# tomwhite/disq

Measured on AMD Instinct MI355X. Metric: decompressed BAM GB/s + reads/sec (whole node) at 1/2/4/8 MI355X, higher is better.
Workload: dtype u8

## Files before the change

disq_amd/csrc/dq_api.hip:

```cpp
#include <hip/hip_runtime.h>

#include <fcntl.h>
#include <sys/stat.h>
#include <unistd.h>

#include <algorithm>
#include <chrono>
#include <cstdio>
#include <cstdlib>
#include <cstring>
#include <map>
#include <string>
#include <thread>
#include <type_traits>
#include <sys/mman.h>
#include <mutex>
#include <vector>

#include "../../include/disq_gpu.h"
#include "dq_internal.h"
#include "dq_sam_core.h"
#include "dq_vcf_core.h"
#include "dq_vcf_gt_core.h"
#include "dq_vcf_info_core.h"
// ... 644 lines not shown
    launch_exclusive_scan_i32(ctx->blk_us.as<int32_t>(), ctx->uoff.as<int64_t>(), nblk,
                              ctx->tmp.as<int64_t>(), s);
    if ((rc = get_i64(ctx, ctx->uoff.as<int64_t>() + nblk, &ulen))) return rc;
  }
  dbg(s, "chain", nblk, broken);
  ctx->nblk = nblk;
  if (nblk == 0 && L > 0) RET(DQ_EFORMAT, "no BGZF blocks found");
  ctx->ulen = ulen;
  HIPCHK(hipEventRecord(ctx->ev[1], s));
  if ((rc = ensure_all(ctx, ctx->U, (size_t)ulen + 256))) return rc;
  if ((rc = ensure_all(ctx, ctx->status, sizeof(int32_t) * (size_t)(nblk + 1)))) return rc;
  HIPCHK(hipMemsetAsync(ctx->status.p, 0, sizeof(int32_t) * (size_t)(nblk + 1), s));
  HIPCHK(hipMemsetAsync(ctx->U.as<uint8_t>() + ulen, 0, 256, s));
  {
    const uint32_t* crc_init = inflate3_tables(ctx->o.device);
    if (!crc_init) RET(DQ_EDEVICE, "CRC32 table initialisation failed on this device");
    static const bool timing = getenv("DQ_TIMING") != nullptr;
    uint64_t* tim = nullptr;
    if (timing) {
      HIPCHK(hipMalloc(&tim, sizeof(uint64_t) * 48 * (size_t)std::max<int64_t>(1, nblk)));
      HIPCHK(hipMemsetAsync(tim, 0, sizeof(uint64_t) * 48 * (size_t)std::max<int64_t>(1, nblk), s));
    }
    HIPCHK(hipEventRecord(ctx->ev[5], s));
    if ((rc = ensure_all(ctx, ctx->tails, INFLATE_TAIL_BYTES * (size_t)std::max<int64_t>(1, nblk)))) return rc;
    launch_inflate3(ctx->cbuf(), ctx->blk_pos.as<int64_t>(), ctx->blk_cs.as<int32_t>(),
                    ctx->blk_us.as<int32_t>(), ctx->uoff.as<int64_t>(), nblk, ctx->U.as<uint8_t>(),
                    ctx->status.as<int32_t>(), ctx->o.verify_crc, crc_init, tim, s, nullptr, 0,
                    ctx->tails.p);
    HIPCHK(hipEventRecord(ctx->ev[6], s));
    if (timing) {
      std::vector<uint64_t> h(48 * (size_t)nblk);
      HIPCHK(hipMemcpyAsync(h.data(), tim, 8 * h.size(), hipMemcpyDeviceToHost, s));
      HIPCHK(hipStreamSynchronize(s));
      (void)hipFree(tim);
      double acc[24] = {0};
      for (int64_t i = 0; i < nblk; i++)
        for (int k = 0; k < 24; k++) acc[k] += (double)h[32 * (size_t)i + k];
      static const char* nm[16] = {"header", "tables", "spec", "rounds", "scan", "emit",
                                   "resolve+store", "crc", "hdr_read_lengths", "resolve_hop_next", "redo_rounds", "tables_build",
                                   "resolve_steps_jumps", "resolve_store", "resolve_jump_tail", "res_batches"};
      fprintf(stderr, "[dq] inflate3 phase cycles per BGZF block (thread 0, s_memtime):");
      for (int k = 0; k < 16; k++)
        if (nm[k][0] != '-') fprintf(stderr, " %s=%.0f", nm[k], acc[k] / (double)std::max<int64_t>(1, nblk));
      fprintf(stderr, "\n");
      const double nb = (double)std::max<int64_t>(1, nblk);
      fprintf(stderr, "[dq] first deflate block: header=%.0f tables=%.0f spec=%.0f rounds=%.0f emit=%.0f; "
              "later ones: header=%.0f tables=%.0f spec=%.0f rounds=%.0f emit=%.0f; deflate blocks per "
// ... 1002 lines not shown
      if (j0 >= nblk || bp[(size_t)j0] != a) RET(DQ_EFORMAT, ".bai chunk does not start at a BGZF block");
      const int64_t jc = std::upper_bound(bp.begin(), bp.end(), e) - bp.begin();
      const int64_t j1 = std::min(nblk, jc + extra);
      if (!win.empty() && j0 <= win.back().j1 + GAP) {
        W& w = win.back();
        w.jc = std::max(w.jc, jc);
        w.j1 = std::max(w.j1, j1);
      } else {
        win.push_back({j0, jc, j1, ub[k]});
      }
    }
    std::vector<int32_t> sel;
    for (const W& w : win)
      for (int64_t j = std::max<int64_t>(w.j0, sel.empty() ? 0 : sel.back() + 1); j < w.j1; j++)
        sel.push_back((int32_t)j);
    const int64_t nsel = (int64_t)sel.size();
    HIPCHK(hipEventRecord(ctx->ev[5], s));
    if (nsel) {
      if ((rc = ensure_all(ctx, ctx->sel, 4 * (size_t)nsel))) return rc;
      HIPCHK(hipMemcpyAsync(ctx->sel.p, sel.data(), 4 * (size_t)nsel, hipMemcpyHostToDevice, s));
      HIPCHK(hipMemsetAsync(ctx->status.p, 0, sizeof(int32_t) * (size_t)(nblk + 1), s));
      const uint32_t* crc_init = inflate3_tables(ctx->o.device);
      if (!crc_init) RET(DQ_EDEVICE, "CRC32 table initialisation failed on this device");
      if ((rc = ensure_all(ctx, ctx->tails, INFLATE_TAIL_BYTES * (size_t)nsel))) return rc;
      launch_inflate3(ctx->cbuf(), ctx->blk_pos.as<int64_t>(), ctx->blk_cs.as<int32_t>(),
                      ctx->blk_us.as<int32_t>(), ctx->uoff.as<int64_t>(), nblk, ctx->U.as<uint8_t>(),
                      ctx->status.as<int32_t>(), ctx->o.verify_crc, crc_init, nullptr, s,
                      ctx->sel.as<int32_t>(), nsel, ctx->tails.p);
    }
    HIPCHK(hipEventRecord(ctx->ev[6], s));
    {
      unsigned long long* d_bad = reinterpret_cast<unsigned long long*>(ctx->scal.as<char>() + 144);
      HIPCHK(hipMemsetAsync(d_bad, 0xff, 8, s));
      if (nsel) launch_first_bad(ctx->status.as<int32_t>(), ctx->sel.as<int32_t>(), nsel, d_bad, s);
      unsigned long long bad = 0;
      HIPCHK(hipMemcpyAsync(&bad, d_bad, 8, hipMemcpyDeviceToHost, s));
      HIPCHK(hipStreamSynchronize(s));
      if (bad != ~0ull) {
        int32_t st = 0;
        HIPCHK(hipMemcpy(&st, ctx->status.as<int32_t>() + bad, 4, hipMemcpyDeviceToHost));
        char msg[256];
        snprintf(msg, sizeof msg, "%s in BGZF block at %lld", status_name(st),
                 (long long)(bp[(size_t)bad] + ctx->base));
        RET(DQ_EFORMAT, msg);
      }
    }
    const int64_t SEG = 64 * 1024;
// ... 2906 lines not shown
```

disq_amd/csrc/dq_inflate3.hip:

```cpp
#include "dq_inflate_core.h"
#include "dq_internal.h"

#include <mutex>
#include <vector>

namespace dq {
namespace {

using namespace dqi;

#define DQ_HD __device__ __host__ __attribute__((always_inline)) inline

#ifndef DQ_BLK_WG
#define DQ_BLK_WG 512
#endif
constexpr int WG = DQ_BLK_WG;
static_assert(WG % 128 == 0 && WG >= 512 && WG <= 1024, "whole waves on every SIMD");
constexpr int NWV = WG / 64;
constexpr int NDEC = WG;
constexpr uint32_t OV_DEFAULT = 96;
#ifndef DQ_TAIL_OV
#define DQ_TAIL_OV OV_DEFAULT
#endif
constexpr int OUTCAP = 65536 + 24;
// ... 46 lines not shown
enum : int32_t { F_EXIT = 0, F_EOB = 1, F_ERR = 2, F_END = 3 };

constexpr int TOUT = 4096;
constexpr int TAIL_MAX_BITS = 32768;
constexpr int TW = 4;
#ifndef DQ_ROOT_REG
#define DQ_ROOT_REG 1
#endif
#ifndef DQ_TAIL_HDR1
#define DQ_TAIL_HDR1 1
#endif
constexpr int T_NCK = 4;
#ifndef DQ_TAIL_SEG
#define DQ_TAIL_SEG 96
#endif
constexpr int TAIL_SEG_MIN = DQ_TAIL_SEG;
constexpr int TIM_W = 32;
struct TailDesc {
  int32_t pos;
  int32_t produced;
  uint32_t crc_raw;
  int32_t flag;
};

struct alignas(16) LdsI {
  static constexpr int kLSUB = T_LSUB, kDROOT = T_DROOT, kDSUB = T_DSUB;
  [[maybe_unused]] static constexpr int kTEND = T_END;
  static constexpr bool kPair = true;
  alignas(8) uint32_t bm[2048];
  union {
    struct {
      uint16_t T[T_END];
      HuffCanon hl, hd;
      uint16_t lend[16], dend[16];
      uint16_t lent[288];
      uint16_t dent[32];
      union {
        uint16_t pair[1 << LR];
        struct {
          uint8_t lens[320];
          uint8_t clen[20];
          uint16_t clt[128];
          union {
            struct {
              int32_t cntw[NWV];
              int32_t cnts[NWV];
// ... 25 lines not shown
    struct {
      int32_t wsum[16];
      int32_t small[8 * 7];
    };
    uint32_t scratch[16 + 8 * 7];
  };
  alignas(16) uint8_t out[OUTCAP];
};
static_assert(sizeof(((LdsI*)nullptr)->scratch) >= 64 * 4, "one emit dummy word per lane");
static_assert(offsetof(LdsI, out) < 65536 - 4096, "the tables' offsets fit the DS offset field");
static_assert(2 * sizeof(LdsI) <= 160 * 1024, "two workgroups per CU");
static_assert(HB_WORDS * 4 <= T_END * 2, "header staging fits the decode table");

__device__ inline uint32_t* emit_dummy(LdsI& L) { return L.scratch; }

__constant__ uint32_t c_crc4[4][256];
__constant__ uint32_t c_x2n[32];
__constant__ uint32_t c_x8n[TOUT + 1];
constexpr int CRC_SL = 4 * (((65536 / 4 + WG - 1) / WG) | 1);
static_assert(CRC_SL * WG >= 65536, "the slices cover the largest block");
__constant__ uint32_t c_slice_shift[WG];
__constant__ uint8_t c_clorder3[19] = {16, 17, 18, 0, 8, 7, 9, 6, 10, 5, 11, 4, 12, 3, 13, 2, 14, 1, 15};

enum { M_ERR = 0, M_SLOW = 1 , M_A = 4, M_LAST, M_MORE, M_MORE1,
       M_LQ0 = 15, M_LQN, M_DQ0, M_DQN, M_NEXT,
       M_LASTF, M_RCNT = 28 ,
       M_DIRTY = 30  };

template <class LT>
__device__ __attribute__((always_inline)) inline void set_err(LT& L, int32_t code) { atomicCAS(&L.misc[M_ERR], 0, code); }


#define DQ_AI __device__ __attribute__((always_inline)) inline

DQ_AI int tid_fresh() {
  int t = (int)threadIdx.x;
  asm volatile("" : "+v"(t));
  return t;
}

typedef uint32_t u32x4 __attribute__((ext_vector_type(4)));
DQ_AI void st_nt(uint4* d, uint4 v) {
  u32x4 x = {v.x, v.y, v.z, v.w};
  __builtin_nontemporal_store(x, reinterpret_cast<u32x4*>(d));
}

struct GSrc {
// ... 737 lines not shown
      tacc[i] += now_ - tlast;                            \
      tlast = now_;                                       \
    }                                                     \
  } while (0)
#define TCOUNT(i) do { if (TIMING && threadIdx.x == 0) tacc[i] += 1; } while (0)
  if ((int64_t)blockIdx.x >= nblk) return;
  const int64_t b = sel ? (int64_t)sel[blockIdx.x] : (int64_t)blockIdx.x;
  const int t = threadIdx.x, lane = t & 63, wv = t >> 6;
  const int64_t cpos = blk_pos[b];
  const int32_t csize = blk_csize[b];
  const int32_t isize = blk_usize[b];
  const int64_t ub = uoff[b];
  const int sh = (int)(ub & 15);
  const uint8_t* dp = C + cpos + 18;
  const int mis = (int)(reinterpret_cast<uintptr_t>(dp) & 15);
  const uint32_t* W =
      reinterpret_cast<const uint32_t*>(__builtin_assume_aligned(dp - mis, 16));
  const uint32_t a0 = 8u * (uint32_t)mis;
  const int32_t dbytes = csize - 26;
  const uint32_t endbits = a0 + 8u * (uint32_t)max(dbytes, 0);

  uint32_t warm = 0;
  if ((sflags & 16) && 128u * (uint32_t)t < (uint32_t)(mis + max(dbytes, 0))) warm = W[32 * t];
  for (int i = t; i < 2048; i += WG) L.bm[i] = 0;
  if (t < 32) L.misc[t] = 0;
  if (t == 0) {
    if (isize < 0 || isize > 65536) L.misc[M_ERR] = ST_ISIZE;
    else if (dbytes < 0) L.misc[M_ERR] = ST_OVERREAD;
  }
  asm volatile("" ::"v"(warm));
  __syncthreads();
  int32_t produced = 0;
  uint32_t pos = a0;
  bool deferred = false;
  while (L.misc[M_ERR] == 0 && produced < isize) {
    const int t = tid_fresh(), lane = t & 63, wv = t >> 6;
    if (t == 0) L.misc[M_SLOW] = 0;
    const uint32_t clpos = pos + 17;
    const uint32_t hbase = clpos >> 5;
    const uint32_t hw = t < HB_WORDS ? W[hbase + t] : 0u;
    const uint32_t hcl = t < 19 ? peek_bits(W, clpos + 3 * t, 3) : 0u;
    const uint32_t h = peek_bits(W, pos, 17);
    const int32_t bfinal = (int32_t)(h & 1), btype = (int32_t)((h >> 1) & 3);
    const int32_t herr = pos + 3 > endbits ? ST_OVERREAD : btype == 3 ? ST_BAD_BLOCKTYPE : 0;
    if (herr) {
      if (t == 0) L.misc[M_ERR] = herr;
      break;
    }
    if (btype == 0) {
      const uint32_t q = (pos + 3 + 7) & ~7u;
      const uint8_t* bp = reinterpret_cast<const uint8_t*>(W) + q / 8;
      const uint32_t len = bp[0] | ((uint32_t)bp[1] << 8), nl = bp[2] | ((uint32_t)bp[3] << 8);
      const int32_t serr = (len ^ 0xffffu) != nl ? ST_BAD_STORED : q + 32 + 8 * len > endbits ? ST_OVERREAD : 0;
      if (serr) {
        if (t == 0) L.misc[M_ERR] = serr;
        break;
      }
      const uint8_t* sp = bp + 4;
      const int32_t n = min((int32_t)len, isize - produced);
      DQ_CHK(sh + produced + n <= OUTCAP, CHK_K2_IMAGE);
      for (int i = t; i < n; i += WG) L.out[sh + produced + i] = sp[i];
      produced += n;
      pos = q + 32 + 8 * len;
      __syncthreads();
      if (bfinal) break;
      continue;
    }
    const int nlen = btype == 1 ? 288 : (int)((h >> 3) & 31) + 257;
    const int ndist = btype == 1 ? 32 : (int)((h >> 8) & 31) + 1;
    if (btype == 2 && (nlen > 286 || ndist > 30)) {
      if (t == 0) L.misc[M_ERR] = ST_BAD_TABLE;
      break;
    }
    if (btype == 1) {
      for (int i = t; i < 320; i += WG) L.u.d.x.h.lens[i] = fixed_len(i);
      if (t == 0) L.misc[M_A] = (int32_t)(pos + 3);
      __syncthreads();
    } else {
      const int ncode = (int)((h >> 13) & 15) + 4;
      for (int i = t; i < 320; i += WG) L.u.d.x.h.lens[i] = 0;
      if (t < HB_WORDS) reinterpret_cast<uint32_t*>(L.u.d.T)[t] = hw;
      if (t < 19) L.u.d.x.h.clen[c_clorder3[t]] = t < ncode ? (uint8_t)hcl : 0;
      __syncthreads();
      if (t < 128) {
        bool ok = true;
        L.u.d.x.h.clt[t] = clt_entry(L.u.d.x.h.clen, t, &ok);
        if (t == 0 && !ok) set_err(L, ST_BAD_TABLE);
      }
      __syncthreads();
      if (L.misc[M_ERR]) break;
      {
        const uint64_t tr0 = TIMING ? __builtin_amdgcn_s_memtime() : 0;
        const uint32_t a = read_lengths(L, clpos + 3 * (uint32_t)ncode, nlen, ndist, endbits, hbase);
        if (t == 0) L.misc[M_A] = (int32_t)a;
        if (TIMING && t == 0) tacc[8] += __builtin_amdgcn_s_memtime() - tr0;
      }
      __syncthreads();
      if (L.misc[M_ERR]) break;
      if (L.u.d.x.h.lens[256] == 0) {
        if (t == 0) L.misc[M_ERR] = ST_BAD_TABLE;
// ... 607 lines not shown
      cr = gf2_mulmod(cshift, cr);
    }
    cr = wave_incl_xor(cr);
    if (lane == 63) L.wsum[wv] = (int32_t)cr;
    __syncthreads();
    if (t == 0) {
      uint32_t x = 0;
      for (int w = 0; w < WG / 64; w++) x ^= (uint32_t)L.wsum[w];
      if (deferred) {
        tails[blockIdx.x].crc_raw = x;
      } else {
        const uint32_t crc = (x ^ cinit) ^ 0xffffffffu;
        if (crc != cwant) status[b] = ST_CRC;
      }
    }
  }
  TST(7);
  if (TIMING && t == 0)
    for (int i = 0; i < 24; i++) tim[(int64_t)blockIdx.x * TIM_W + i] = tacc[i];
  if (TIMING && t == 0)
    for (int i = 0; i < 7; i++) tim[(int64_t)blockIdx.x * TIM_W + 24 + i] = (uint64_t)L.misc[21 + i];
}

struct alignas(16) LdsW {
  static constexpr int kLSUB = 0, kDROOT = 1 << LR, kDSUB = 0, kTEND = (1 << LR) + (1 << DR);
  static constexpr bool kPair = false;
  union {
    struct {
      uint16_t T[kTEND];
      HuffCanon hl, hd;
      uint16_t lend[16], dend[16];
      uint16_t lent[288];
      uint16_t dent[32];
      union {
        struct {
          uint8_t lens[320];
          uint8_t clen[20];
          uint16_t clt[128];
          int32_t cnt[32];
          int32_t run[32];
        } h;
      } x;
    } d;
    uint32_t crc4[4][256];
  } u;
  alignas(16) uint8_t out[TOUT + 32];
// ... 218 lines not shown
  const int32_t csize = blk_csize[b];
  const int32_t isize = blk_usize[b];
  const int64_t ub = uoff[b];
  const int32_t p0 = td.produced;
  const int sh = (int)((ub + p0) & 15);
  const uint8_t* dp = C + cpos + 18;
  const int mis = (int)(reinterpret_cast<uintptr_t>(dp) & 15);
  const uint32_t* W = reinterpret_cast<const uint32_t*>(__builtin_assume_aligned(dp - mis, 16));
  const int32_t dbytes = csize - 26;
  const uint32_t endbits = 8u * (uint32_t)mis + 8u * (uint32_t)max(dbytes, 0);
#ifdef DQ_CHECKED
  GSrc gsrc{W, (endbits >> 5) + 8, 4u << 12};
#else
  const GSrc gsrc{W};
#endif
  uint32_t warm = 0;
  {
    const uint32_t lo = (uint32_t)td.pos >> 3, nbytes = endbits / 8 - min(endbits / 8, lo);
    if ((uint32_t)lane * 128 < nbytes)
      warm = *reinterpret_cast<const uint32_t*>(reinterpret_cast<const uint8_t*>(W) + ((lo + 128 * lane) & ~3u));
  }
  for (int i = lane; i < TOUT / 32; i += 64) L.bm[i] = 0;
  if (lane < 8) L.misc[lane] = 0;
  __builtin_amdgcn_wave_barrier();
  int32_t produced = p0;
  uint32_t pos = (uint32_t)td.pos;
  uint64_t tph[5] = {0, 0, 0, 0, 0};
  uint64_t tl = TIMING ? __builtin_amdgcn_s_memtime() : 0;
  auto tick = [&](int k) {
    if (TIMING) {
      const uint64_t now = __builtin_amdgcn_s_memtime();
      tph[k] += now - tl;
      tl = now;
    }
  };
  while (L.misc[M_ERR] == 0 && produced < isize) {
    const uint32_t clpos = pos + 17;
    const uint32_t hbase = clpos >> 5;
#if DQ_TAIL_HDR1
    constexpr int HWN = (HB_WORDS + 63) / 64;
    uint32_t hw[HWN];
#pragma unroll
    for (int j = 0; j < HWN; j++) hw[j] = lane + 64 * j < HB_WORDS ? W[hbase + lane + 64 * j] : 0u;
    const uint32_t clv = lane < 19 ? peek_bits(W, clpos + 3 * (uint32_t)lane, 3) : 0u;
#endif
    const uint32_t h = peek_bits(W, pos, 17);
    const int32_t bfinal = (int32_t)(h & 1), btype = (int32_t)((h >> 1) & 3);
    const int32_t herr = pos + 3 > endbits ? ST_OVERREAD : btype == 3 ? ST_BAD_BLOCKTYPE : 0;
    if (herr) {
      set_err(L, herr);
      break;
    }
    if (btype == 0) {
      const uint32_t q = (pos + 3 + 7) & ~7u;
      const uint8_t* bp = reinterpret_cast<const uint8_t*>(W) + q / 8;
      const uint32_t len = bp[0] | ((uint32_t)bp[1] << 8), nl = bp[2] | ((uint32_t)bp[3] << 8);
      const int32_t serr = (len ^ 0xffffu) != nl ? ST_BAD_STORED : q + 32 + 8 * len > endbits ? ST_OVERREAD : 0;
      if (serr) {
        set_err(L, serr);
        break;
      }
      const int32_t n = min((int32_t)len, isize - produced);
      if (produced + n - p0 > TOUT) {
        set_err(L, ST_SHORT);
        break;
      }
      for (int i = lane; i < n; i += 64) L.out[sh + produced - p0 + i] = bp[4 + i];
      produced += n;
      pos = q + 32 + 8 * len;
      __builtin_amdgcn_wave_barrier();
      if (bfinal) break;
      continue;
    }
    const int nlen = btype == 1 ? 288 : (int)((h >> 3) & 31) + 257;
    const int ndist = btype == 1 ? 32 : (int)((h >> 8) & 31) + 1;
    if (btype == 2 && (nlen > 286 || ndist > 30)) {
      set_err(L, ST_BAD_TABLE);
      break;
    }
    uint32_t a;
    if (btype == 1) {
      for (int i = lane; i < 320; i += 64) L.u.d.x.h.lens[i] = fixed_len(i);
      a = pos + 3;
    } else {
      const int ncode = (int)((h >> 13) & 15) + 4;
      for (int i = lane; i < 320; i += 64) L.u.d.x.h.lens[i] = 0;
#if DQ_TAIL_HDR1
#pragma unroll
      for (int j = 0; j < HWN; j++)
        if (lane + 64 * j < HB_WORDS) reinterpret_cast<uint32_t*>(L.u.d.T)[lane + 64 * j] = hw[j];
      if (lane < 19) L.u.d.x.h.clen[c_clorder3[lane]] = lane < ncode ? (uint8_t)clv : 0;
#else
      for (int i = lane; i < HB_WORDS; i += 64) reinterpret_cast<uint32_t*>(L.u.d.T)[i] = W[hbase + i];
      if (lane < 19)
        L.u.d.x.h.clen[c_clorder3[lane]] = lane < ncode ? (uint8_t)peek_bits(W, clpos + 3 * lane, 3) : 0;
#endif
      __builtin_amdgcn_wave_barrier();
      bool ok = true;
      L.u.d.x.h.clt[lane] = clt_entry(L.u.d.x.h.clen, lane, &ok);
      L.u.d.x.h.clt[lane + 64] = clt_entry(L.u.d.x.h.clen, lane + 64, &ok);
      if (__any(!ok)) {
        set_err(L, ST_BAD_TABLE);
        break;
      }
      __builtin_amdgcn_wave_barrier();
      a = read_lengths_wave(L, clpos + 3 * (uint32_t)ncode, nlen, ndist, endbits, hbase);
      __builtin_amdgcn_wave_barrier();
      if (L.misc[M_ERR]) break;
      if (L.u.d.x.h.lens[256] == 0) {
        set_err(L, ST_BAD_TABLE);
        break;
      }
    }
    tick(0);
    build_tables_wave(L, nlen, ndist);
    if (L.misc[M_ERR]) break;
    __builtin_amdgcn_wave_barrier();
    const bool slow = L.misc[M_SLOW] != 0;
    if (a > endbits) {
      set_err(L, ST_OVERREAD);
      break;
    }
    tick(1);
    const uint32_t span = endbits - a;
    const int nl = (int)max(1u, min(64u, span / (uint32_t)TAIL_SEG_MIN));
    const uint32_t seg = (span + nl - 1) / nl;
    const bool act = lane < nl;
    const uint32_t sB = a + (uint32_t)lane * seg;
    const uint32_t sE = lane == nl - 1 ? 0xffffffffu : sB + seg;
    int32_t AB = -1, AE = 0, AC = 0, SE = 0, SC = 0;
    if (act) {
      const uint32_t start = lane == 0 ? a : (sB > a + OV ? sB - OV : a);
      for (int j = 0; j < T_NCK; j++) L.ck[j * 64 + lane] = 0xffffffffu;
      int32_t B = -1, E = 0, c = 0;
// ... 321 lines not shown
  if (device < 0 || device >= kMaxDevices) return nullptr;
  DevTables& D = g_dev[device];
  std::call_once(D.once, [&] {
    static const HostTables H;
    int prev = -1;
    (void)hipGetDevice(&prev);
    bool ok = hipSetDevice(device) == hipSuccess;
    ok = ok && hipMemcpyToSymbol(HIP_SYMBOL(c_crc4), H.crc4, sizeof H.crc4) == hipSuccess;
    ok = ok && hipMemcpyToSymbol(HIP_SYMBOL(c_slice_shift), H.slice, sizeof H.slice) == hipSuccess;
    ok = ok && hipMemcpyToSymbol(HIP_SYMBOL(c_x2n), H.x2n, sizeof H.x2n) == hipSuccess;
    ok = ok && hipMemcpyToSymbol(HIP_SYMBOL(c_x8n), H.x8n, sizeof H.x8n) == hipSuccess;
    ok = ok && hipMalloc(&D.crc_init, sizeof(uint32_t) * H.init.size()) == hipSuccess;
    ok = ok && hipMemcpy(D.crc_init, H.init.data(), sizeof(uint32_t) * H.init.size(),
                         hipMemcpyHostToDevice) == hipSuccess;
    D.ok = ok;
    if (prev >= 0) (void)hipSetDevice(prev);
  });
  return D.ok ? D.crc_init : nullptr;
}

void launch_inflate3(const uint8_t* C, const int64_t* blk_pos, const int32_t* blk_csize,
                     const int32_t* blk_usize, const int64_t* uoff, int64_t nblk, uint8_t* U,
                     int32_t* status, int32_t verify_crc, const uint32_t* crc_init, uint64_t* tim,
                     hipStream_t s, const int32_t* sel, int64_t nsel, void* tails_buf) {
  if (nblk <= 0) return;
  const int64_t ngrid = sel ? nsel : nblk;
  if (ngrid <= 0) return;
#ifdef DQ_TUNING
  static const uint32_t ov = getenv("DQ_OV") ? (uint32_t)atoi(getenv("DQ_OV")) : OV_DEFAULT;
  static const uint32_t sflags =
      (getenv("DQ_STORE") ? (uint32_t)atoi(getenv("DQ_STORE")) & 3u : 2u) |
      (getenv("DQ_NDEC") ? (uint32_t)(atoi(getenv("DQ_NDEC")) & 1023) << 8 : 0u) |
      (getenv("DQ_SEGBITS") ? (uint32_t)(atoi(getenv("DQ_SEGBITS")) & 1023) << 20 : 0u) |
      (getenv("DQ_WARM") && atoi(getenv("DQ_WARM")) ? 16u : 0u);
  static const unsigned ldspad = getenv("DQ_LDSPAD") ? (unsigned)atoi(getenv("DQ_LDSPAD")) : 0u;
  static const bool tail_on = !getenv("DQ_TAIL") || atoi(getenv("DQ_TAIL")) != 0;
#else
  constexpr uint32_t ov = OV_DEFAULT;
  constexpr uint32_t sflags = 2u;
  constexpr unsigned ldspad = 0u;
  constexpr bool tail_on = true;
#endif
  TailDesc* td = tail_on ? static_cast<TailDesc*>(tails_buf) : nullptr;
  if (td) (void)hipMemsetAsync(td, 0, sizeof(TailDesc) * (size_t)ngrid, s);
#define DQ_LAUNCH(TM, NBT, GT)                                                                  \
  hipLaunchKernelGGL((inflate_block_kernel<TM, NBT, GT>), dim3((unsigned)ngrid), dim3(WG), ldspad, s, C, \
                     blk_pos, blk_csize, blk_usize, uoff, ngrid, U, status, verify_crc, crc_init, tim, ov, \
                     sflags, sel, td)
  if (tim)
    DQ_LAUNCH(true, DQ_RES_NB, DQ_RES_G);
  else
    DQ_LAUNCH(false, DQ_RES_NB, DQ_RES_G);
#undef DQ_LAUNCH
  if (td && tim)
    hipLaunchKernelGGL((inflate_tail_kernel<true>), dim3((unsigned)((ngrid + TW - 1) / TW)), dim3(64 * TW), 0, s,
                       C, blk_pos, blk_csize, blk_usize, uoff, ngrid, U, status, verify_crc, crc_init,
                       ov == OV_DEFAULT ? (uint32_t)DQ_TAIL_OV : ov, sflags, sel, td, tim + TIM_W * ngrid);
  else if (td)
    hipLaunchKernelGGL((inflate_tail_kernel<false>), dim3((unsigned)((ngrid + TW - 1) / TW)), dim3(64 * TW), 0, s,
                       C, blk_pos, blk_csize, blk_usize, uoff, ngrid, U, status, verify_crc, crc_init,
                       ov == OV_DEFAULT ? (uint32_t)DQ_TAIL_OV : ov, sflags, sel, td, nullptr);
}

}
```

disq_amd/csrc/dq_internal.h:

```cpp
#pragma once
#include <hip/hip_runtime.h>
#include <stdint.h>

enum : int32_t {
  ST_OK = 0,
  ST_BAD_HEADER = 1,
  ST_BAD_BLOCKTYPE = 2,
  ST_BAD_STORED = 3,
  ST_BAD_TABLE = 4,
  ST_BAD_CODE = 5,
  ST_BAD_DIST = 6,
  ST_SHORT = 7,
  ST_OVERREAD = 8,
  ST_CRC = 9,
  ST_ISIZE = 10,
  ST_HANG = 11,
  ST_TEXT_START = 12,
};

enum : int {
  CHK_K1_SLOT = 0,
  CHK_K2_BITS = 1,
  CHK_K2_IMAGE = 2,
  CHK_K2_TABLE = 3,
// ... 76 lines not shown
void launch_gather_slots(const Cand* slots, const int32_t* counts, const int64_t* offs,
                         int64_t nchunks, Cand* out, int64_t cap, const int32_t* over_map,
                         const Cand* big, hipStream_t s);
void launch_valid_flags(const Cand* cand, const int64_t* ncand, int64_t cap, int32_t* flags,
                        hipStream_t s);
void launch_chain2(const uint8_t* C, int64_t L, const Cand* cand, const int64_t* ncand, int64_t cap,
                   const int64_t* voff, int64_t* blk_pos, int32_t* blk_csize, int32_t* blk_usize,
                   int64_t blk_cap, int64_t* d_nblk, int32_t* d_broken, int32_t eof_in_buf,
                   hipStream_t s);
void launch_chain_check(const Cand* cand, const int64_t* d_ncand, int64_t cap, const int64_t* blk_pos,
                        const int64_t* d_nblk, unsigned long long* out, hipStream_t s);
void launch_first_bad(const int32_t* status, const int32_t* sel, int64_t n, unsigned long long* out,
                      hipStream_t s);
void launch_chain_serial(const uint8_t* C, int64_t clen, int64_t start, int64_t* blk_pos,
                         int32_t* blk_csize, int32_t* blk_usize, int64_t cap, int64_t* d_nblk,
                         int32_t* d_status, hipStream_t s);

void launch_exclusive_scan_i32(const int32_t* in, int64_t* out, int64_t n, int64_t* tmp,
                               hipStream_t s);
void launch_exclusive_scan_i64(const int64_t* in, int64_t* out, int64_t n, int64_t* tmp,
                               hipStream_t s);

const uint32_t* inflate3_tables(int device);
constexpr size_t INFLATE_TAIL_BYTES = 16;
void launch_inflate3(const uint8_t* C, const int64_t* blk_pos, const int32_t* blk_csize,
                     const int32_t* blk_usize, const int64_t* uoff, int64_t nblk, uint8_t* U,
                     int32_t* status, int32_t verify_crc, const uint32_t* crc_init, uint64_t* tim,
                     hipStream_t s, const int32_t* sel, int64_t nsel, void* tails);

void launch_block_stats(const int64_t* blk_pos, const int32_t* blk_cs, const int64_t* uoff,
                        int64_t nblk, int64_t ulen, int64_t x, uint64_t* out, hipStream_t s);

constexpr int64_t SPLIT_FROM_SBI = -2;
struct SplitPlan {
  int64_t split_start, split_end;
  int64_t first_blk;
  int64_t u_lo, u_hi;
  int64_t rec_lin;
  uint64_t vstart, vend;
  int32_t status;
  int32_t rec_span;
};
void launch_plan_blocks(const Cand* cand, const int64_t* d_ncand, const int64_t* blk_pos,
                        const int32_t* blk_usize, const int64_t* uoff, const int64_t* d_nblk,
                        SplitPlan* plans, int64_t nsplit, hipStream_t s);
void launch_guess_all(const uint8_t* U, int64_t ulen, int32_t u_is_eof, const int32_t* ref_len,
                      int32_t n_ref, uint8_t* flag, hipStream_t s);
void launch_first_record(const uint8_t* U, int64_t ulen, int32_t u_is_eof, const int32_t* ref_len,
                         int32_t n_ref, const int64_t* blk_pos, const int64_t* uoff,
                         const int64_t* d_nblk, SplitPlan* plans, int64_t nsplit,
                         unsigned long long* best, hipStream_t s);
// ... 296 lines not shown
```

Measured before the change: 191.4.

## Decode dynamic Huffman headers in a one-lane-per-block prepass kernel

Adds a separate kernel that decodes each BGZF block's first dynamic-Huffman deflate header with one lane per block. It stores the code lengths packed as nibbles, plus the header end position and status, in an enlarged per-block scratch buffer. The block and tail inflate kernels load these precomputed lengths and skip the workgroup-wide serial header parse for the first deflate block. This takes the serial header decode off the critical path of the 512-thread workgroups, at the cost of two extra kernel launches, more scratch memory and extra global traffic.

```diff
diff --git a/disq_amd/csrc/dq_api.hip b/disq_amd/csrc/dq_api.hip
--- a/disq_amd/csrc/dq_api.hip
+++ b/disq_amd/csrc/dq_api.hip
@@ -690,7 +690,7 @@
       HIPCHK(hipMemsetAsync(tim, 0, sizeof(uint64_t) * 48 * (size_t)std::max<int64_t>(1, nblk), s));
     }
     HIPCHK(hipEventRecord(ctx->ev[5], s));
-    if ((rc = ensure_all(ctx, ctx->tails, INFLATE_TAIL_BYTES * (size_t)std::max<int64_t>(1, nblk)))) return rc;
+    if ((rc = ensure_all(ctx, ctx->tails, INFLATE_SCRATCH_BYTES * (size_t)std::max<int64_t>(1, nblk)))) return rc;
     launch_inflate3(ctx->cbuf(), ctx->blk_pos.as<int64_t>(), ctx->blk_cs.as<int32_t>(),
                     ctx->blk_us.as<int32_t>(), ctx->uoff.as<int64_t>(), nblk, ctx->U.as<uint8_t>(),
                     ctx->status.as<int32_t>(), ctx->o.verify_crc, crc_init, tim, s, nullptr, 0,
@@ -1739,7 +1739,7 @@
       HIPCHK(hipMemsetAsync(ctx->status.p, 0, sizeof(int32_t) * (size_t)(nblk + 1), s));
       const uint32_t* crc_init = inflate3_tables(ctx->o.device);
       if (!crc_init) RET(DQ_EDEVICE, "CRC32 table initialisation failed on this device");
-      if ((rc = ensure_all(ctx, ctx->tails, INFLATE_TAIL_BYTES * (size_t)nsel))) return rc;
+      if ((rc = ensure_all(ctx, ctx->tails, INFLATE_SCRATCH_BYTES * (size_t)nsel))) return rc;
       launch_inflate3(ctx->cbuf(), ctx->blk_pos.as<int64_t>(), ctx->blk_cs.as<int32_t>(),
                       ctx->blk_us.as<int32_t>(), ctx->uoff.as<int64_t>(), nblk, ctx->U.as<uint8_t>(),
                       ctx->status.as<int32_t>(), ctx->o.verify_crc, crc_init, nullptr, s,
diff --git a/disq_amd/csrc/dq_hdr_core.h b/disq_amd/csrc/dq_hdr_core.h
--- /dev/null
+++ b/disq_amd/csrc/dq_hdr_core.h
@@ -0,0 +1,147 @@
+#pragma once
+#include <stdint.h>
+
+#ifndef __HIPCC__
+#ifndef __host__
+#define __host__
+#define __device__
+#endif
+#endif
+
+#define DQH_INLINE __host__ __device__ inline __attribute__((always_inline))
+
+namespace dqh {
+
+enum : int32_t {
+  HDR_NONE = 0,
+  HDR_DYN = 1,
+  HDR_ERR = 2,
+};
+constexpr int32_t HDR_BAD_TABLE = 4, HDR_OVERREAD = 8;
+constexpr uint32_t HDR_WORDS = 160;
+constexpr int HDR_LENS = 320;
+
+struct HdrInfo {
+  int32_t kind, status;
+  int32_t nlen, ndist, bfinal;
+  uint32_t end;
+};
+
+template <class Src>
+struct Bits {
+  uint64_t bb;
+  uint32_t bc, wp;
+  DQH_INLINE void init(const Src& S, uint32_t pos) {
+    const uint32_t wi = pos >> 5, sh = pos & 31;
+    bb = (((uint64_t)S.word(wi + 1) << 32) | S.word(wi)) >> sh;
+    bc = 64 - sh;
+    wp = wi + 2;
+  }
+  DQH_INLINE void fill(const Src& S) {
+    if (bc <= 32) {
+      bb |= (uint64_t)S.word(wp) << bc;
+      bc += 32;
+      wp += 1;
+    }
+  }
+  DQH_INLINE uint32_t peek() const { return (uint32_t)bb; }
+  DQH_INLINE void skip(uint32_t n) {
+    bb >>= n;
+    bc -= n;
+  }
+  DQH_INLINE uint32_t pos() const { return wp * 32 - bc; }
+};
+
+template <class Src, class Tbl, class Sink>
+DQH_INLINE HdrInfo hdr_decode(const Src& S, Tbl& T, Sink& K, uint32_t pos, uint32_t endbits) {
+  constexpr uint8_t order[19] = {16, 17, 18, 0, 8, 7, 9, 6, 10, 5, 11, 4, 12, 3, 13, 2, 14, 1, 15};
+  HdrInfo R = {HDR_NONE, 0, 0, 0, 0, pos};
+  if (pos + 3 > endbits) return R;
+  Bits<Src> B;
+  B.init(S, pos);
+  const uint32_t h = B.peek();
+  R.bfinal = (int32_t)(h & 1);
+  if (((h >> 1) & 3) != 2) return R;
+  R.nlen = (int32_t)((h >> 3) & 31) + 257;
+  R.ndist = (int32_t)((h >> 8) & 31) + 1;
+  const int ncode = (int)((h >> 13) & 15) + 4;
+  B.skip(17);
+  R.kind = HDR_ERR;
+  R.status = HDR_BAD_TABLE;
+  if (R.nlen > 286 || R.ndist > 30) return R;
+  if (pos + 17 + 3 * (uint32_t)ncode > endbits) {
+    R.status = HDR_OVERREAD;
+    return R;
+  }
+  uint64_t cl = 0, cnt = 0;
+  for (int i = 0; i < 19; i++) {
+    B.fill(S);
+    const uint32_t v = i < ncode ? B.peek() & 7 : 0;
+    B.skip(i < ncode ? 3 : 0);
+    cl |= (uint64_t)v << (3 * order[i]);
+    cnt += 1ull << (8 * v);
+  }
+  uint64_t nxt = 0;
+  {
+    int left = 1;
+    uint32_t code = 0;
+    bool ok = true;
+    for (int l = 1; l <= 7; l++) {
+      const int c = (int)((cnt >> (8 * l)) & 0xff);
+      left = 2 * left - c;
+      ok = ok && left >= 0;
+      nxt |= (uint64_t)(code & 0xff) << (8 * l);
+      code = (code + (uint32_t)c) << 1;
+    }
+    if (!ok || left != 0) return R;
+  }
+  for (int s = 0; s < 19; s++) {
+    const uint32_t l = (uint32_t)(cl >> (3 * s)) & 7;
+    if (l == 0) continue;
+    const uint32_t c = (uint32_t)(nxt >> (8 * l)) & 0xff;
+    nxt += 1ull << (8 * l);
+    uint32_t r = 0;
+    for (uint32_t i = 0; i < l; i++) r |= ((c >> i) & 1u) << (l - 1 - i);
+    for (uint32_t k = r & 127; k < 128; k += 1u << l) T.set(k, (uint32_t)s << 3 | l);
+  }
+  const int total = R.nlen + R.ndist;
+  int have = 0, prev = -1;
+  bool eob = false;
+  for (int it = 0; it < 316 && have < total; it++) {
+    if (B.pos() > endbits) {
+      R.status = HDR_OVERREAD;
+      return R;
+    }
+    B.fill(S);
+    const uint32_t v = B.peek();
+    const uint32_t e = T.get(v & 127);
+    const uint32_t len = e & 7, sy = e >> 3;
+    if (len == 0) return R;
+    const uint32_t ex = sy < 16 ? 0u : sy == 16 ? 2u : sy == 17 ? 3u : 7u;
+    const int xv = (int)((v >> len) & ((1u << ex) - 1));
+    B.skip(len + ex);
+    const int rep = sy < 16 ? 1 : sy == 18 ? 11 + xv : 3 + xv;
+    const int val = sy < 16 ? (int)sy : sy == 16 ? prev : 0;
+    if (val < 0) return R;
+    if (have + rep > total) return R;
+    if (val != 0)
+      for (int i = have; i < have + rep; i++) {
+        K.put((uint32_t)(i < R.nlen ? i : 288 + i - R.nlen), (uint32_t)val);
+        eob = eob || i == 256;
+      }
+    have += rep;
+    prev = val;
+  }
+  if (have < total) return R;
+  R.end = B.pos();
+  if (R.end > endbits) {
+    R.status = HDR_OVERREAD;
+    return R;
+  }
+  if (!eob) return R;
+  R.kind = HDR_DYN;
+  R.status = 0;
+  return R;
+}
+
+}
diff --git a/disq_amd/csrc/dq_inflate3.hip b/disq_amd/csrc/dq_inflate3.hip
--- a/disq_amd/csrc/dq_inflate3.hip
+++ b/disq_amd/csrc/dq_inflate3.hip
@@ -1,3 +1,4 @@
+#include "dq_hdr_core.h"
 #include "dq_inflate_core.h"
 #include "dq_internal.h"
 
@@ -92,6 +93,26 @@
   uint32_t crc_raw;
   int32_t flag;
 };
+
+#ifndef DQ_HDR_PREPASS
+#define DQ_HDR_PREPASS 1
+#endif
+constexpr int HDR_LW = dqh::HDR_LENS / 8;
+struct alignas(16) HdrMeta {
+  uint32_t info;
+  uint32_t end;
+  uint32_t pad[2];
+};
+static_assert(sizeof(TailDesc) + sizeof(HdrMeta) + 4 * HDR_LW == INFLATE_SCRATCH_BYTES, "scratch per block");
+DQ_HD int hm_kind(uint32_t info) { return (int)(info & 3u); }
+DQ_HD int32_t hm_bfinal(uint32_t info) { return (int32_t)((info >> 2) & 1u); }
+DQ_HD int hm_ndist(uint32_t info) { return (int)((info >> 3) & 31u); }
+DQ_HD int hm_nlen(uint32_t info) { return (int)((info >> 8) & 511u); }
+DQ_HD int32_t hm_status(uint32_t info) { return (int32_t)(info >> 24); }
+DQ_HD uint32_t nib4(uint32_t x) {
+  x = (x | (x << 8)) & 0x00ff00ffu;
+  return (x | (x << 4)) & 0x0f0f0f0fu;
+}
 
 struct alignas(16) LdsI {
   static constexpr int kLSUB = T_LSUB, kDROOT = T_DROOT, kDSUB = T_DSUB;
@@ -163,7 +184,8 @@
 __constant__ uint32_t c_slice_shift[WG];
 __constant__ uint8_t c_clorder3[19] = {16, 17, 18, 0, 8, 7, 9, 6, 10, 5, 11, 4, 12, 3, 13, 2, 14, 1, 15};
 
-enum { M_ERR = 0, M_SLOW = 1 , M_A = 4, M_LAST, M_MORE, M_MORE1,
+enum { M_ERR = 0, M_SLOW = 1 ,
+       M_HDR = 2 , M_A = 4, M_LAST, M_MORE, M_MORE1,
        M_LQ0 = 15, M_LQN, M_DQ0, M_DQN, M_NEXT,
        M_LASTF, M_RCNT = 28 ,
        M_DIRTY = 30  };
@@ -947,11 +969,27 @@
 
   uint32_t warm = 0;
   if ((sflags & 16) && 128u * (uint32_t)t < (uint32_t)(mis + max(dbytes, 0))) warm = W[32 * t];
+  const bool hon = (sflags & 32) != 0;
+  uint32_t hinfo = 0;
+  if (hon) {
+    const HdrMeta* hrec = reinterpret_cast<const HdrMeta*>(tails + nblk);
+    const HdrMeta* hm = hrec + blockIdx.x + (tid_fresh() >> 10);
+    hinfo = hm->info;
+    if (hm_kind(hinfo) == dqh::HDR_DYN && t < HDR_LW) {
+      const uint32_t w = reinterpret_cast<const uint32_t*>(hrec + nblk)[(int64_t)blockIdx.x * HDR_LW + t];
+      uint32_t* l8 = reinterpret_cast<uint32_t*>(L.u.d.x.h.lens);
+      l8[2 * t] = nib4(w & 0xffffu);
+      l8[2 * t + 1] = nib4(w >> 16);
+    }
+    if (t == M_A) L.misc[M_A] = (int32_t)hm->end;
+    if (t == M_HDR) L.misc[M_HDR] = hm_kind(hinfo) == dqh::HDR_DYN ? (int32_t)hinfo : 0;
+  }
   for (int i = t; i < 2048; i += WG) L.bm[i] = 0;
-  if (t < 32) L.misc[t] = 0;
+  if (t < 32 && !(hon && (t == M_A || t == M_HDR))) L.misc[t] = 0;
   if (t == 0) {
     if (isize < 0 || isize > 65536) L.misc[M_ERR] = ST_ISIZE;
     else if (dbytes < 0) L.misc[M_ERR] = ST_OVERREAD;
+    else if (isize > 0 && hm_kind(hinfo) == dqh::HDR_ERR) L.misc[M_ERR] = hm_status(hinfo);
   }
   asm volatile("" ::"v"(warm));
   __syncthreads();
@@ -963,8 +1001,9 @@
     if (t == 0) L.misc[M_SLOW] = 0;
     const uint32_t clpos = pos + 17;
     const uint32_t hbase = clpos >> 5;
-    const uint32_t hw = t < HB_WORDS ? W[hbase + t] : 0u;
-    const uint32_t hcl = t < 19 ? peek_bits(W, clpos + 3 * t, 3) : 0u;
+    const bool hpre = L.misc[M_HDR] != 0;
+    const uint32_t hw = !hpre && t < HB_WORDS ? W[hbase + t] : 0u;
+    const uint32_t hcl = !hpre && t < 19 ? peek_bits(W, clpos + 3 * t, 3) : 0u;
     const uint32_t h = peek_bits(W, pos, 17);
     const int32_t bfinal = (int32_t)(h & 1), btype = (int32_t)((h >> 1) & 3);
     const int32_t herr = pos + 3 > endbits ? ST_OVERREAD : btype == 3 ? ST_BAD_BLOCKTYPE : 0;
@@ -1001,6 +1040,9 @@
       for (int i = t; i < 320; i += WG) L.u.d.x.h.lens[i] = fixed_len(i);
       if (t == 0) L.misc[M_A] = (int32_t)(pos + 3);
       __syncthreads();
+    } else if (hpre) {
+      __syncthreads();
+      if (t == 0) L.misc[M_HDR] = 0;
     } else {
       const int ncode = (int)((h >> 13) & 15) + 4;
       for (int i = t; i < 320; i += WG) L.u.d.x.h.lens[i] = 0;
@@ -1654,6 +1696,81 @@
     for (int i = 0; i < 7; i++) tim[(int64_t)blockIdx.x * TIM_W + 24 + i] = (uint64_t)L.misc[21 + i];
 }
 
+constexpr int HP_LS = 65;
+struct HpSrc {
+  const uint32_t* __restrict__ W;
+  uint32_t last;
+  DQ_AI uint32_t word(uint32_t i) const {
+    return *reinterpret_cast<const uint32_t*>(reinterpret_cast<const uint8_t*>(W) + (min(i, last) << 2));
+  }
+};
+struct HpTbl {
+  uint8_t* t;
+  DQ_AI void set(uint32_t k, uint32_t v) { t[k * 64] = (uint8_t)v; }
+  DQ_AI uint32_t get(uint32_t k) const { return t[k * 64]; }
+};
+struct HpSink {
+  uint32_t* w;
+  uint32_t cur, acc;
+  DQ_AI void put(uint32_t i, uint32_t v) {
+    if ((i >> 3) != cur) {
+      flush();
+      cur = i >> 3;
+      acc = 0;
+    }
+    acc |= v << (4 * (i & 7));
+  }
+  DQ_AI void flush() {
+    if (acc) w[cur * HP_LS] = acc;
+  }
+};
+
+template <bool TAIL>
+__global__ __launch_bounds__(64) void inflate_header_kernel(
+    const uint8_t* __restrict__ C, const int64_t* __restrict__ blk_pos,
+    const int32_t* __restrict__ blk_csize, int64_t ngrid, const int32_t* __restrict__ sel,
+    const TailDesc* __restrict__ tails, HdrMeta* __restrict__ hdr) {
+  __shared__ uint8_t clt[128 * 64];
+  __shared__ uint32_t lw[HDR_LW * HP_LS];
+  const int lane = (int)threadIdx.x;
+  const int64_t i0 = (int64_t)blockIdx.x * 64, i = i0 + lane;
+  bool act = i < ngrid;
+  uint32_t pos = 0;
+  if (TAIL && act) {
+    const TailDesc td = tails[i];
+    act = td.flag == 1;
+    pos = (uint32_t)td.pos;
+  }
+  for (int w = 0; w < HDR_LW; w++) lw[w * HP_LS + lane] = 0;
+  dqh::HdrInfo R = {dqh::HDR_NONE, 0, 0, 0, 0, 0};
+  if (act) {
+    const int64_t b = sel ? (int64_t)sel[i] : i;
+    const uint8_t* dp = C + blk_pos[b] + 18;
+    const int mis = (int)(reinterpret_cast<uintptr_t>(dp) & 15);
+    const uint32_t a0 = 8u * (uint32_t)mis;
+    const uint32_t endbits = a0 + 8u * (uint32_t)max(blk_csize[b] - 26, 0);
+    if (!TAIL) pos = a0;
+    const HpSrc S{reinterpret_cast<const uint32_t*>(dp - mis), (pos >> 5) + dqh::HDR_WORDS - 1};
+    HpTbl T{clt + lane};
+    HpSink K{lw + lane, 0, 0};
+    R = dqh::hdr_decode(S, T, K, pos, endbits);
+    K.flush();
+    HdrMeta m;
+    m.info = (uint32_t)R.kind | (uint32_t)R.bfinal << 2 | (uint32_t)(R.ndist & 31) << 3 |
+             (uint32_t)(R.nlen & 511) << 8 | (uint32_t)R.status << 24;
+    m.end = R.end;
+    m.pad[0] = m.pad[1] = 0;
+    hdr[i] = m;
+  }
+  __syncthreads();
+  const uint64_t dyn = __ballot(R.kind == dqh::HDR_DYN);
+  uint32_t* out = reinterpret_cast<uint32_t*>(hdr + ngrid) + i0 * HDR_LW;
+  for (int k = 0; k < HDR_LW; k++) {
+    const int g = 64 * k + lane, r = g / HDR_LW, w = g - r * HDR_LW;
+    if ((dyn >> r) & 1) out[g] = lw[w * HP_LS + r];
+  }
+}
+
 struct alignas(16) LdsW {
   static constexpr int kLSUB = 0, kDROOT = 1 << LR, kDSUB = 0, kTEND = (1 << LR) + (1 << DR);
   static constexpr bool kPair = false;
@@ -1918,6 +2035,21 @@
   }
   for (int i = lane; i < TOUT / 32; i += 64) L.bm[i] = 0;
   if (lane < 8) L.misc[lane] = 0;
+  uint32_t hinfo = 0, hend = 0;
+  if (sflags & 32) {
+    const HdrMeta* hdr = reinterpret_cast<const HdrMeta*>(tails + ngrid);
+    const HdrMeta hm = hdr[gi];
+    hinfo = hm.info;
+    hend = hm.end;
+    if (hm_kind(hinfo) == dqh::HDR_DYN && lane < HDR_LW) {
+      const uint32_t w = reinterpret_cast<const uint32_t*>(hdr + ngrid)[gi * HDR_LW + lane];
+      uint32_t* l8 = reinterpret_cast<uint32_t*>(L.u.d.x.h.lens);
+      l8[2 * lane] = nib4(w & 0xffffu);
+      l8[2 * lane + 1] = nib4(w >> 16);
+    }
+    if (hm_kind(hinfo) == dqh::HDR_ERR && lane == 0) L.misc[M_ERR] = hm_status(hinfo);
+  }
+  const bool hpre = hm_kind(hinfo) == dqh::HDR_DYN;
   __builtin_amdgcn_wave_barrier();
   int32_t produced = p0;
   uint32_t pos = (uint32_t)td.pos;
@@ -1931,81 +2063,91 @@
     }
   };
   while (L.misc[M_ERR] == 0 && produced < isize) {
-    const uint32_t clpos = pos + 17;
-    const uint32_t hbase = clpos >> 5;
+    int nlen, ndist;
+    int32_t bfinal;
+    uint32_t a;
+    if (hpre && pos == (uint32_t)td.pos) {
+      nlen = hm_nlen(hinfo);
+      ndist = hm_ndist(hinfo);
+      bfinal = hm_bfinal(hinfo);
+      a = hend;
+    } else {
+      const uint32_t clpos = pos + 17;
+      const uint32_t hbase = clpos >> 5;
 #if DQ_TAIL_HDR1
-    constexpr int HWN = (HB_WORDS + 63) / 64;
-    uint32_t hw[HWN];
-#pragma unroll
-    for (int j = 0; j < HWN; j++) hw[j] = lane + 64 * j < HB_WORDS ? W[hbase + lane + 64 * j] : 0u;
-    const uint32_t clv = lane < 19 ? peek_bits(W, clpos + 3 * (uint32_t)lane, 3) : 0u;
-#endif
-    const uint32_t h = peek_bits(W, pos, 17);
-    const int32_t bfinal = (int32_t)(h & 1), btype = (int32_t)((h >> 1) & 3);
-    const int32_t herr = pos + 3 > endbits ? ST_OVERREAD : btype == 3 ? ST_BAD_BLOCKTYPE : 0;
-    if (herr) {
-      set_err(L, herr);
-      break;
-    }
-    if (btype == 0) {
-      const uint32_t q = (pos + 3 + 7) & ~7u;
-      const uint8_t* bp = reinterpret_cast<const uint8_t*>(W) + q / 8;
-      const uint32_t len = bp[0] | ((uint32_t)bp[1] << 8), nl = bp[2] | ((uint32_t)bp[3] << 8);
-      const int32_t serr = (len ^ 0xffffu) != nl ? ST_BAD_STORED : q + 32 + 8 * len > endbits ? ST_OVERREAD : 0;
-      if (serr) {
-        set_err(L, serr);
+      constexpr int HWN = (HB_WORDS + 63) / 64;
+      uint32_t hw[HWN];
+#pragma unroll
+      for (int j = 0; j < HWN; j++) hw[j] = lane + 64 * j < HB_WORDS ? W[hbase + lane + 64 * j] : 0u;
+      const uint32_t clv = lane < 19 ? peek_bits(W, clpos + 3 * (uint32_t)lane, 3) : 0u;
+#endif
+      const uint32_t h = peek_bits(W, pos, 17);
+      bfinal = (int32_t)(h & 1);
+      const int32_t btype = (int32_t)((h >> 1) & 3);
+      const int32_t herr = pos + 3 > endbits ? ST_OVERREAD : btype == 3 ? ST_BAD_BLOCKTYPE : 0;
+      if (herr) {
+        set_err(L, herr);
         break;
       }
-      const int32_t n = min((int32_t)len, isize - produced);
-      if (produced + n - p0 > TOUT) {
-        set_err(L, ST_SHORT);
-        break;
-      }
-      for (int i = lane; i < n; i += 64) L.out[sh + produced - p0 + i] = bp[4 + i];
-      produced += n;
-      pos = q + 32 + 8 * len;
-      __builtin_amdgcn_wave_barrier();
-      if (bfinal) break;
-      continue;
-    }
-    const int nlen = btype == 1 ? 288 : (int)((h >> 3) & 31) + 257;
-    const int ndist = btype == 1 ? 32 : (int)((h >> 8) & 31) + 1;
-    if (btype == 2 && (nlen > 286 || ndist > 30)) {
-      set_err(L, ST_BAD_TABLE);
-      break;
-    }
-    uint32_t a;
-    if (btype == 1) {
-      for (int i = lane; i < 320; i += 64) L.u.d.x.h.lens[i] = fixed_len(i);
-      a = pos + 3;
-    } else {
-      const int ncode = (int)((h >> 13) & 15) + 4;
-      for (int i = lane; i < 320; i += 64) L.u.d.x.h.lens[i] = 0;
-#if DQ_TAIL_HDR1
-#pragma unroll
-      for (int j = 0; j < HWN; j++)
-        if (lane + 64 * j < HB_WORDS) reinterpret_cast<uint32_t*>(L.u.d.T)[lane + 64 * j] = hw[j];
-      if (lane < 19) L.u.d.x.h.clen[c_clorder3[lane]] = lane < ncode ? (uint8_t)clv : 0;
-#else
-      for (int i = lane; i < HB_WORDS; i += 64) reinterpret_cast<uint32_t*>(L.u.d.T)[i] = W[hbase + i];
-      if (lane < 19)
-        L.u.d.x.h.clen[c_clorder3[lane]] = lane < ncode ? (uint8_t)peek_bits(W, clpos + 3 * lane, 3) : 0;
-#endif
-      __builtin_amdgcn_wave_barrier();
-      bool ok = true;
-      L.u.d.x.h.clt[lane] = clt_entry(L.u.d.x.h.clen, lane, &ok);
-      L.u.d.x.h.clt[lane + 64] = clt_entry(L.u.d.x.h.clen, lane + 64, &ok);
-      if (__any(!ok)) {
+      if (btype == 0) {
+        const uint32_t q = (pos + 3 + 7) & ~7u;
+        const uint8_t* bp = reinterpret_cast<const uint8_t*>(W) + q / 8;
+        const uint32_t len = bp[0] | ((uint32_t)bp[1] << 8), nl = bp[2] | ((uint32_t)bp[3] << 8);
+        const int32_t serr = (len ^ 0xffffu) != nl ? ST_BAD_STORED : q + 32 + 8 * len > endbits ? ST_OVERREAD : 0;
+        if (serr) {
+          set_err(L, serr);
+          break;
+        }
+        const int32_t n = min((int32_t)len, isize - produced);
+        if (produced + n - p0 > TOUT) {
+          set_err(L, ST_SHORT);
+          break;
+        }
+        for (int i = lane; i < n; i += 64) L.out[sh + produced - p0 + i] = bp[4 + i];
+        produced += n;
+        pos = q + 32 + 8 * len;
+        __builtin_amdgcn_wave_barrier();
+        if (bfinal) break;
+        continue;
+      }
+      nlen = btype == 1 ? 288 : (int)((h >> 3) & 31) + 257;
+      ndist = btype == 1 ? 32 : (int)((h >> 8) & 31) + 1;
+      if (btype == 2 && (nlen > 286 || ndist > 30)) {
         set_err(L, ST_BAD_TABLE);
         break;
       }
-      __builtin_amdgcn_wave_barrier();
-      a = read_lengths_wave(L, clpos + 3 * (uint32_t)ncode, nlen, ndist, endbits, hbase);
-      __builtin_amdgcn_wave_barrier();
-      if (L.misc[M_ERR]) break;
-      if (L.u.d.x.h.lens[256] == 0) {
-        set_err(L, ST_BAD_TABLE);
-        break;
+      if (btype == 1) {
+        for (int i = lane; i < 320; i += 64) L.u.d.x.h.lens[i] = fixed_len(i);
+        a = pos + 3;
+      } else {
+        const int ncode = (int)((h >> 13) & 15) + 4;
+        for (int i = lane; i < 320; i += 64) L.u.d.x.h.lens[i] = 0;
+#if DQ_TAIL_HDR1
+#pragma unroll
+        for (int j = 0; j < HWN; j++)
+          if (lane + 64 * j < HB_WORDS) reinterpret_cast<uint32_t*>(L.u.d.T)[lane + 64 * j] = hw[j];
+        if (lane < 19) L.u.d.x.h.clen[c_clorder3[lane]] = lane < ncode ? (uint8_t)clv : 0;
+#else
+        for (int i = lane; i < HB_WORDS; i += 64) reinterpret_cast<uint32_t*>(L.u.d.T)[i] = W[hbase + i];
+        if (lane < 19)
+          L.u.d.x.h.clen[c_clorder3[lane]] = lane < ncode ? (uint8_t)peek_bits(W, clpos + 3 * lane, 3) : 0;
+#endif
+        __builtin_amdgcn_wave_barrier();
+        bool ok = true;
+        L.u.d.x.h.clt[lane] = clt_entry(L.u.d.x.h.clen, lane, &ok);
+        L.u.d.x.h.clt[lane + 64] = clt_entry(L.u.d.x.h.clen, lane + 64, &ok);
+        if (__any(!ok)) {
+          set_err(L, ST_BAD_TABLE);
+          break;
+        }
+        __builtin_amdgcn_wave_barrier();
+        a = read_lengths_wave(L, clpos + 3 * (uint32_t)ncode, nlen, ndist, endbits, hbase);
+        __builtin_amdgcn_wave_barrier();
+        if (L.misc[M_ERR]) break;
+        if (L.u.d.x.h.lens[256] == 0) {
+          set_err(L, ST_BAD_TABLE);
+          break;
+        }
       }
     }
     tick(0);
@@ -2373,7 +2515,7 @@
 void launch_inflate3(const uint8_t* C, const int64_t* blk_pos, const int32_t* blk_csize,
                      const int32_t* blk_usize, const int64_t* uoff, int64_t nblk, uint8_t* U,
                      int32_t* status, int32_t verify_crc, const uint32_t* crc_init, uint64_t* tim,
-                     hipStream_t s, const int32_t* sel, int64_t nsel, void* tails_buf) {
+                     hipStream_t s, const int32_t* sel, int64_t nsel, void* scratch) {
   if (nblk <= 0) return;
   const int64_t ngrid = sel ? nsel : nblk;
   if (ngrid <= 0) return;
@@ -2392,25 +2534,34 @@
   constexpr unsigned ldspad = 0u;
   constexpr bool tail_on = true;
 #endif
-  TailDesc* td = tail_on ? static_cast<TailDesc*>(tails_buf) : nullptr;
+  TailDesc* td = tail_on ? static_cast<TailDesc*>(scratch) : nullptr;
+  HdrMeta* hm = DQ_HDR_PREPASS && td ? reinterpret_cast<HdrMeta*>(td + ngrid) : nullptr;
+  const uint32_t kflags = sflags | (hm ? 32u : 0u);
   if (td) (void)hipMemsetAsync(td, 0, sizeof(TailDesc) * (size_t)ngrid, s);
+  const dim3 hgrid((unsigned)((ngrid + 63) / 64));
+  if (hm)
+    hipLaunchKernelGGL((inflate_header_kernel<false>), hgrid, dim3(64), 0, s, C, blk_pos, blk_csize, ngrid, sel,
+                       (const TailDesc*)nullptr, hm);
 #define DQ_LAUNCH(TM, NBT, GT)                                                                  \
   hipLaunchKernelGGL((inflate_block_kernel<TM, NBT, GT>), dim3((unsigned)ngrid), dim3(WG), ldspad, s, C, \
                      blk_pos, blk_csize, blk_usize, uoff, ngrid, U, status, verify_crc, crc_init, tim, ov, \
-                     sflags, sel, td)
+                     kflags, sel, td)
   if (tim)
     DQ_LAUNCH(true, DQ_RES_NB, DQ_RES_G);
   else
     DQ_LAUNCH(false, DQ_RES_NB, DQ_RES_G);
 #undef DQ_LAUNCH
+  if (td && hm)
+    hipLaunchKernelGGL((inflate_header_kernel<true>), hgrid, dim3(64), 0, s, C, blk_pos, blk_csize, ngrid, sel,
+                       (const TailDesc*)td, hm);
   if (td && tim)
     hipLaunchKernelGGL((inflate_tail_kernel<true>), dim3((unsigned)((ngrid + TW - 1) / TW)), dim3(64 * TW), 0, s,
                        C, blk_pos, blk_csize, blk_usize, uoff, ngrid, U, status, verify_crc, crc_init,
-                       ov == OV_DEFAULT ? (uint32_t)DQ_TAIL_OV : ov, sflags, sel, td, tim + TIM_W * ngrid);
+                       ov == OV_DEFAULT ? (uint32_t)DQ_TAIL_OV : ov, kflags, sel, td, tim + TIM_W * ngrid);
   else if (td)
     hipLaunchKernelGGL((inflate_tail_kernel<false>), dim3((unsigned)((ngrid + TW - 1) / TW)), dim3(64 * TW), 0, s,
                        C, blk_pos, blk_csize, blk_usize, uoff, ngrid, U, status, verify_crc, crc_init,
-                       ov == OV_DEFAULT ? (uint32_t)DQ_TAIL_OV : ov, sflags, sel, td, nullptr);
-}
-
-}
+                       ov == OV_DEFAULT ? (uint32_t)DQ_TAIL_OV : ov, kflags, sel, td, nullptr);
+}
+
+}
diff --git a/disq_amd/csrc/dq_internal.h b/disq_amd/csrc/dq_internal.h
--- a/disq_amd/csrc/dq_internal.h
+++ b/disq_amd/csrc/dq_internal.h
@@ -122,11 +122,11 @@
                                hipStream_t s);
 
 const uint32_t* inflate3_tables(int device);
-constexpr size_t INFLATE_TAIL_BYTES = 16;
+constexpr size_t INFLATE_SCRATCH_BYTES = 16 + 16 + 160;
 void launch_inflate3(const uint8_t* C, const int64_t* blk_pos, const int32_t* blk_csize,
                      const int32_t* blk_usize, const int64_t* uoff, int64_t nblk, uint8_t* U,
                      int32_t* status, int32_t verify_crc, const uint32_t* crc_init, uint64_t* tim,
-                     hipStream_t s, const int32_t* sel, int64_t nsel, void* tails);
+                     hipStream_t s, const int32_t* sel, int64_t nsel, void* scratch);
 
 void launch_block_stats(const int64_t* blk_pos, const int32_t* blk_cs, const int64_t* uoff,
                         int64_t nblk, int64_t ulen, int64_t x, uint64_t* out, hipStream_t s);
```

After: 197.5, median of 6. +3.2%, better.
